# Firstastor/polars-quant

Hardware: AMD Instinct MI355X
Metric: indicator+backtest rows/sec, 5000 sym x 2520 day f64 OHLCV (higher is better)
Workload: dtype f64

## Files before the change

polars_quant_amd/csrc/pattern.hip:

```cpp
#include "pq_dev.h"

struct Cdl {
    double o, h, l, c;
    double body, us, ls, mx, mn;
    bool bull, bear, lng, sht, doji, lus, lds, sus, sds, vsus, vsds, vlds;
    __device__ void set(double o_, double h_, double l_, double c_) {
        o = o_; h = h_; l = l_; c = c_;
        bull = c > o;
        bear = c < o;
        body = fabs(o - c);
        mn = fmin(o, c);
        mx = fmax(o, c);
        us = h - mx;
        ls = mn - l;
        lng = body > 0.05 * (o + c) * 0.5;
        sht = body < 0.1 * (o + c) * 0.5;
        doji = body <= 0.005 * (o + c) * 0.5;
        lus = us > 2.0 * body;
        lds = ls > 2.0 * body;
        sus = us < 0.5 * body;
        sds = ls < 0.5 * body;
        vsus = us < 0.1 * body;
        vsds = ls < 0.1 * body;
        vlds = ls > 3.0 * body;
    }
    __device__ bool maru() const { return lng && vsus && vsds; }
};
__device__ __forceinline__ bool nearq(double a, double b, const Cdl &k) { return fabs(a - b) < 0.01 * (k.h + k.l) * 0.5; }
__device__ __forceinline__ bool equalq(double a, double b, const Cdl &k) { return fabs(a - b) < 0.001 * (k.h + k.l) * 0.5; }
__device__ __forceinline__ int pm(bool up, bool dn) { return up ? 100 : (dn ? -100 : 0); }

__device__ __forceinline__ int cdl_eval(int id, const Cdl &a, const Cdl &b, const Cdl &c, const Cdl &d, const Cdl &e, double pen,
                                        int *lookback) {
    switch (id) {
    case 0: *lookback = 2;
        return (c.bull & c.lng & b.bear & b.o > c.c & a.bear & a.o > b.o & a.o < b.c & a.c > c.o & a.c < c.c) ? -100 : 0;
    case 1: *lookback = 2;
        return (c.bear & c.lng & b.bear & b.lng & a.bear & a.lng & b.o < c.o & b.o > c.c & a.o < b.o & a.o > b.c &
                b.c < c.c & a.c < b.c) ? -100 : 0;
    case 2: *lookback = 2;
        return pm(c.bear & c.lng & b.bull & b.c < c.o & b.o > c.c & a.bull & a.c > c.o,
                  c.bull & c.lng & b.bear & b.o < c.c & b.c > c.o & a.bear & a.c < c.o);
    case 3: *lookback = 3;
        return pm(d.bear & c.bear & b.bear & c.c < d.c & b.c < c.c & c.o > d.c & c.o < d.o & b.o > c.c & b.o < c.o &
                      a.bull & a.o < b.c & a.c > d.o,
                  d.bull & c.bull & b.bull & c.c > d.c & b.c > c.c & c.o < d.c & c.o > d.o & b.o < c.c & b.o > c.o &
                      a.bear & a.o > b.c & a.c < d.o);
    case 4: *lookback = 2;
        return pm(c.bear & b.bull & b.o <= c.c & b.c >= c.o & a.bull & a.c > b.c,
                  c.bull & b.bear & b.o >= c.c & b.c <= c.o & a.bear & a.c < b.c);
    case 5: *lookback = 2;
        return (c.bear & c.lng & c.lds & b.bear & b.l > c.l & b.c > c.c & a.bear & a.sht & a.h < b.h & a.l > b.l) ? 100 : 0;
    case 6: *lookback = 2;
        return (c.bull & c.lng & b.bull & b.lng & a.bull & a.lng & b.o > c.o & b.o <= c.c & a.o > b.o & a.o <= b.c &
                b.c > c.c & a.c > b.c) ? 100 : 0;
    case 7: *lookback = 2;
        return pm(c.bear & c.lng & b.doji & b.h < c.l & a.bull & a.l > b.h,
                  c.bull & c.lng & b.doji & b.l > c.h & a.bear & a.h < b.l);
    case 8: *lookback = 2;
        return (c.bull & c.lng & b.bull & a.bull & b.o > c.o & b.o <= c.c & a.o > b.o & a.o <= b.c & b.c > c.c &
                a.c > b.c & a.body < b.body) ? -100 : 0;
    case 9: *lookback = 0;
        return pm(a.bull & a.lng & a.vsds, a.bear & a.lng & a.vsus);
    case 10: *lookback = 4;
        return pm(e.bear & e.lng & d.bear & d.o < e.c & c.c < d.c & a.bull & a.c > d.o & a.c < e.c,
                  e.bull & e.lng & d.bull & d.o > e.c & c.c > d.c & a.bear & a.c < d.o & a.c > e.c);
    case 11: *lookback = 0;
        return pm(a.bull & a.lng & a.vsus, a.bear & a.lng & a.vsds);
    case 12: *lookback = 3;
        return (d.bear & d.lng & d.vsus & d.vsds & c.bear & c.lng & c.vsus & c.vsds & c.c < d.c & b.bear &
                b.h > c.c & a.bear & a.lng & a.o > b.h & a.c < c.l) ? 100 : 0;
    case 13: *lookback = 1;
        return pm(b.bear & b.lng & a.bull & a.lng & nearq(a.c, b.c, a), b.bull & b.lng & a.bear & a.lng & nearq(a.c, b.c, a));
    case 14: *lookback = 1;
        return (b.bull & b.lng & a.bear & a.o > b.c & a.c < (b.c - (b.body * pen)) & a.c > b.o) ? -100 : 0;
    case 15: *lookback = 0;
        return a.doji ? 100 : 0;
    case 16: { *lookback = 1;
        double mid = (a.o + a.c) / 2.0;
        return pm(b.bear & b.lng & a.doji & mid < b.c, b.bull & b.lng & a.doji & mid > b.c); }
    case 17: *lookback = 0;
        return (a.doji & a.lds & a.vsus) ? 100 : 0;
    case 18: *lookback = 1;
        return pm(b.bear & a.bull & a.o <= b.c & a.c >= b.o & (a.o < b.c | a.c > b.o),
                  b.bull & a.bear & a.o >= b.c & a.c <= b.o & (a.o > b.c | a.c < b.o));
    case 19: *lookback = 2;
        return (c.bull & c.lng & b.doji & b.mn > c.c & a.bear & a.c < (c.c - (c.body * pen))) ? -100 : 0;
    case 20: *lookback = 2;
        return (c.bull & c.lng & b.sht & b.mn > c.c & a.bear & a.c < (c.c - (c.body * pen))) ? -100 : 0;
    case 21: { *lookback = 2;
        bool common = b.bull & a.bull & nearq(a.body, b.body, a) & nearq(a.o, b.o, a);
        return pm(c.bull & b.o > c.c & common, c.bear & b.c < c.c & common); }
    case 22: *lookback = 0;
        return (a.doji & a.lus & a.vsds) ? -100 : 0;
    case 23: *lookback = 1;
        return (a.sht & a.ls > (2.0 * a.body) & a.vsus & b.bear) ? 100 : 0;
    case 24: *lookback = 1;
        return (a.sht & a.ls > (2.0 * a.body) & a.vsus & b.bull) ? -100 : 0;
    case 25: *lookback = 1;
        return pm(b.bear & b.lng & a.bull & a.sht & a.o > b.c & a.c < b.o, b.bull & b.lng & a.bear & a.sht & a.o < b.c & a.c > b.o);
    case 26: *lookback = 1;
        return pm(b.bear & b.lng & a.doji & a.mx < b.o & a.mn > b.c, b.bull & b.lng & a.doji & a.mx < b.c & a.mn > b.o);
    case 27: { *lookback = 0;
        bool m = a.sht & a.lus & a.lds;
        return pm(m & a.bull, m & a.bear); }
    case 28: { *lookback = 2;
        bool inside = b.h < c.h & b.l > c.l;
        return pm(inside & a.c > c.h & a.bull, inside & a.c < c.l & a.bear); }
    case 29: { *lookback = 3;
        bool inside = c.h < d.h & c.l > d.l & b.h < c.h & b.l > c.l;
        return pm(inside & a.c > d.h & a.bull, inside & a.c < d.l & a.bear); }
    case 30: *lookback = 1;
        return (b.bear & b.lng & a.bear & a.sht & a.o < b.o & a.c > b.c) ? 100 : 0;
    case 31: *lookback = 2;
        return (c.bear & c.lng & b.bear & b.lng & a.bear & a.lng & equalq(b.o, c.c, a) & equalq(a.o, b.c, a) &
                b.c < c.c & a.c < b.c) ? -100 : 0;
    case 32: *lookback = 1;
        return (b.bear & b.lng & a.bull & a.o < b.c & nearq(a.c, b.c, a)) ? -100 : 0;
    case 33: *lookback = 1;
        return (a.sht & a.us > (2.0 * a.body) & a.vsds & b.bear) ? 100 : 0;
    case 34: *lookback = 1;
        return pm(b.bear & b.maru() & a.bull & a.maru() & a.o > b.o, b.bull & b.maru() & a.bear & a.maru() & a.o < b.o);
    case 35: { *lookback = 1;
        bool bk = b.bear & b.maru() & a.bull & a.maru() & a.o > b.o;
        bool sk = b.bull & b.maru() & a.bear & a.maru() & a.o < b.o;
        bool longer = a.body >= b.body;
        bool bl = bk & longer, sl = sk & longer;
        return pm(bl | (bk & !sl), sl | (sk & !bl)); }
    case 36: *lookback = 4;
        return (e.bear & e.lng & d.bear & d.c < e.c & c.bear & c.c < d.c & b.bear & b.lus & a.bull & a.o > b.o) ? 100 : 0;
    case 37: *lookback = 0;
        return (a.doji & a.lus & a.lds) ? 100 : 0;
    case 38: { *lookback = 0;
        bool m = a.lng & a.sus & a.sds;
        return pm(m & a.bull, m & a.bear); }
    case 39: { *lookback = 0;
        bool m = a.maru();
        return pm(m & a.bull, m & a.bear); }
    case 40: *lookback = 1;
        return (b.bear & b.lng & a.bear & equalq(a.c, b.c, a)) ? 100 : 0;
    case 41: *lookback = 4;
        return (e.bull & e.lng & d.sht & d.o > e.c & c.sht & b.sht & d.l > e.o & c.l > e.o & b.l > e.o & a.bull &
                a.c > e.c) ? 100 : 0;
    case 42: *lookback = 2;
        return (c.bear & c.lng & b.doji & b.mx < c.c & a.bull & a.c > (c.c + (c.body * pen))) ? 100 : 0;
    case 43: *lookback = 2;
        return (c.bear & c.lng & b.sht & b.mx < c.c & a.bull & a.c > (c.c + (c.body * pen))) ? 100 : 0;
    case 44: *lookback = 1;
        return (b.bear & b.lng & a.bull & a.o < b.c & nearq(a.c, b.l, a)) ? -100 : 0;
    case 45: *lookback = 1;
        return (b.bear & b.lng & a.bull & a.o < b.c & a.c > (b.c + (b.body * pen)) & a.c < b.o) ? 100 : 0;
    case 46: *lookback = 0;
        return (a.doji & a.lus & a.lds & nearq(a.us, a.ls, a)) ? 100 : 0;
    case 47: { *lookback = 4;
        bool mid = d.sht & c.sht & b.sht & d.h < e.h & c.h < e.h & b.h < e.h & d.l > e.l & c.l > e.l & b.l > e.l;
        return pm(e.bull & e.lng & mid & a.bull & a.lng & a.c > e.c, e.bear & e.lng & mid & a.bear & a.lng & a.c < e.c); }
    case 48: *lookback = 1;
        return pm(b.bear & b.lng & a.bull & a.lng & equalq(a.o, b.o, a), b.bull & b.lng & a.bear & a.lng & equalq(a.o, b.o, a));
    case 49: *lookback = 1;
        return (a.sht & a.us > (2.0 * a.body) & a.vsds & b.bull) ? -100 : 0;
    case 50: { *lookback = 0;
        bool m = a.sht & a.sus & a.sds;
        return pm(m & a.bull, m & a.bear); }
    case 51: { *lookback = 0;
        bool m = a.sht & a.us > a.body & a.ls > a.body;
        return pm(m & a.bull, m & a.bear); }
    case 52: *lookback = 2;
        return (c.bull & c.lng & b.bull & b.lng & b.c > c.c & a.bull & a.sht & a.c > b.c & a.o > b.o & a.o <= b.c) ? -100 : 0;
    case 53: *lookback = 2;
        return (c.bear & c.lng & b.bull & b.lng & b.o > c.c & a.bear & a.lng & equalq(a.c, c.c, a)) ? 100 : 0;
    case 54: *lookback = 0;
        return (a.doji & a.vlds & a.vsus) ? 100 : 0;
    case 55: *lookback = 2;
        return pm(c.bull & b.bull & b.o > c.c & a.bear & a.o > b.o & a.o < b.c & a.c > c.o & a.c < c.c,
                  c.bear & b.bear & b.o < c.c & a.bull & a.o < b.o & a.o > b.c & a.c < c.o & a.c > c.c);
    case 56: { *lookback = 1;
        double midpoint = b.c + (b.body * 0.5);
        return (b.bear & b.lng & a.bull & a.o < b.c & a.c > b.c & a.c < midpoint) ? -100 : 0; }
    case 57: { *lookback = 2;
        bool dj = c.doji & b.doji & a.doji;
        double m1 = (c.o + c.c) / 2.0, m2 = (b.o + b.c) / 2.0, m3 = (a.o + a.c) / 2.0;
        return pm(dj & m2 < m1 & m3 > m2, dj & m2 > m1 & m3 < m2); }
    case 58: *lookback = 2;
        return (c.bear & c.lng & b.bear & b.l < c.l & b.c > b.l & b.o < c.o & b.o > c.c & a.bull & a.sht & a.c < b.c) ? 100 : 0;
    case 59: *lookback = 2;
        return (c.bull & c.lng & b.bear & b.o > c.c & b.c > c.c & a.bear & a.o > b.o & a.c > c.c & a.c < b.c) ? -100 : 0;
    case 60: *lookback = 2;
        return pm(c.bull & b.bull & b.o > c.c & a.bear & a.o < b.c & a.o > b.o & a.c > c.o & a.c < c.c,
                  c.bear & b.bear & b.o < c.c & a.bull & a.o > b.c & a.o < b.o & a.c < c.o & a.c > c.c);
    }
    *lookback = 0;
    return 0;
}

struct CdlArgs {
    const double *o, *h, *l, *c;
    int32_t *out[PQ_N_PATTERNS];
    double pen[PQ_N_PATTERNS];
};

__device__ __forceinline__ Cdl load_candle(const CdlArgs &a, int64_t base, int64_t q) {
    Cdl k;
    if (q >= 0) k.set(a.o[base + q], a.h[base + q], a.l[base + q], a.c[base + q]);
    else k.set(0.0, 0.0, 0.0, 0.0);
    return k;
}

#ifndef PQ_CDL_R
#define PQ_CDL_R 1
#endif
constexpr int CDL_R = PQ_CDL_R;
template <bool ALL, bool VEC>
__global__ __launch_bounds__(ROW_BLOCK) void cdl_all_kernel(CdlArgs a, Dims d) {
    const int64_t s = blockIdx.y;
    const int64_t t0 = ((int64_t)blockIdx.x * ROW_BLOCK + threadIdx.x) * CDL_R;
    const int64_t slen = dims_len(d, s);
    if (t0 >= slen) return;
    const int64_t base = dims_base(d, s);
#ifndef PQ_CDL_PRIO
#define PQ_CDL_PRIO 0
#endif
    __builtin_amdgcn_s_setprio(PQ_CDL_PRIO);
    Cdl w[CDL_R + 4];
#pragma unroll
    for (int k = 0; k < CDL_R + 4; k++) {
        const int64_t q = t0 + CDL_R - 1 - k;
        w[k] = load_candle(a, base, q < slen ? q : slen - 1);
    }
#pragma unroll
    for (int id = 0; id < PQ_N_PATTERNS; id++) {
        if (!ALL && a.out[id] == nullptr) continue;
        int v[CDL_R];
#pragma unroll
        for (int r = 0; r < CDL_R; r++) {
            int lb;
            const int x = cdl_eval(id, w[CDL_R - 1 - r], w[CDL_R - r], w[CDL_R + 1 - r], w[CDL_R + 2 - r], w[CDL_R + 3 - r], a.pen[id], &lb);
            v[r] = (t0 + r >= lb) ? x : 0;
        }
#if PQ_EXP_NOSTORE_ON
        if (v[0] == 123456789) a.out[id][base + t0] = v[0];
#else
        int32_t *dst = &a.out[id][base + t0];
        if (VEC && (CDL_R == 1 || t0 + CDL_R <= slen)) {
            typedef int pq_irv __attribute__((ext_vector_type(CDL_R)));
            pq_irv vv;
#pragma unroll
            for (int r = 0; r < CDL_R; r++) vv[r] = v[r];
            __builtin_nontemporal_store(vv, reinterpret_cast<pq_irv *>(dst));
        } else {
#pragma unroll
            for (int r = 0; r < CDL_R; r++)
                if (t0 + r < slen) __builtin_nontemporal_store(v[r], dst + r);
        }
#endif
    }
}

__global__ __launch_bounds__(ROW_BLOCK) void cdl_one_kernel(CdlArgs a, int id, Dims d) {
    const int64_t s = blockIdx.y;
    const int64_t t = (int64_t)blockIdx.x * ROW_BLOCK + threadIdx.x;
    if (t >= dims_len(d, s)) return;
    const int64_t base = dims_base(d, s);
    Cdl w[5];
#pragma unroll
    for (int k = 0; k < 5; k++) w[k] = load_candle(a, base, t - k);
    int lb;
    int v = cdl_eval(id, w[0], w[1], w[2], w[3], w[4], a.pen[0], &lb);
    a.out[0][base + t] = (t >= lb) ? v : 0;
}

static const char *const k_pattern_names[PQ_N_PATTERNS] = {
    "cdl2crows", "cdl3blackcrows", "cdl3inside", "cdl3linestrike", "cdl3outside", "cdl3starsinsouth",
    "cdl3whitesoldiers", "cdlabandonedbaby", "cdladvanceblock", "cdlbelthold", "cdlbreakaway",
    "cdlclosingmarubozu", "cdlconcealbabyswall", "cdlcounterattack", "cdldarkcloudcover", "cdldoji",
    "cdldojistar", "cdldragonflydoji", "cdlengulfing", "cdleveningdojistar", "cdleveningstar",
    "cdlgapsidesidewhite", "cdlgravestonedoji", "cdlhammer", "cdlhangingman", "cdlharami", "cdlharamicross",
    "cdlhighwave", "cdlhikkake", "cdlhikkakemod", "cdlhomingpigeon", "cdlidentical3crows", "cdlinneck",
    "cdlinvertedhammer", "cdlkicking", "cdlkickingbylength", "cdlladderbottom", "cdllongleggeddoji",
    "cdllongline", "cdlmarubozu", "cdlmatchinglow", "cdlmathold", "cdlmorningdojistar", "cdlmorningstar",
    "cdlonneck", "cdlpiercing", "cdlrickshawman", "cdlrisefall3methods", "cdlseparatinglines",
    "cdlshootingstar", "cdlshortline", "cdlspinningtop", "cdlstalledpattern", "cdlsticksandwich", "cdltakuri",
    "cdltasukigap", "cdlthrusting", "cdltristar", "cdlunique3river", "cdlupsidegap2crows",
    "cdlxsidegap3methods"};

#include <string.h>
extern "C" {

const char *pq_pattern_name(int32_t id) { return (id >= 0 && id < PQ_N_PATTERNS) ? k_pattern_names[id] : nullptr; }
int32_t pq_pattern_id(const char *name) {
    if (!name) return -1;
    for (int i = 0; i < PQ_N_PATTERNS; i++)
        if (strcmp(name, k_pattern_names[i]) == 0) return i;
    return -1;
}

struct CdlBlob {
    CdlArgs args;
    int id;
    pq_batch b;
};
static void cdl_launch_blob(const void *blob, hipStream_t stream);
static pq_status cdl_launch(pq_ctx *ctx, const pq_batch *b, const CdlArgs &args, int id) {
    if (b->n_series == 0 || b->len == 0) return PQ_OK;
    CdlBlob cb{args, id, *b};
    if (ctx->rec) {
        static_assert(sizeof(CdlBlob) <= sizeof(RowThunk::blob), "CdlBlob too large");
        RowThunk t;
        t.launch = &cdl_launch_blob;
        t.row_id = 0;
        t.blob_bytes = (int)sizeof cb;
        t.dims = dims_of(b);
        memcpy(t.blob, &cb, sizeof cb);
        t.n_reads = 4;
        t.reads[0] = args.o; t.reads[1] = args.h; t.reads[2] = args.l; t.reads[3] = args.c;
        t.n_writes = 0;
        for (int i = 0; i < PQ_N_PATTERNS; i++) if (args.out[i]) t.writes[t.n_writes++] = args.out[i];
        return rec_add_row(ctx, t);
    }
    cdl_launch_blob(&cb, ctx->stream);
    PQ_HIP_TRY(hipGetLastError());
    return PQ_OK;
}
static void cdl_launch_blob(const void *blob, hipStream_t stream) {
    const CdlBlob &cb = *reinterpret_cast<const CdlBlob *>(blob);
    const pq_batch *b = &cb.b;
    const CdlArgs &args = cb.args;
    const int id = cb.id;
    for (int64_t s0 = 0; s0 < b->n_series; s0 += 65535) {
        int64_t ns = b->n_series - s0 < 65535 ? b->n_series - s0 : 65535;
        CdlArgs a2 = args;
        int64_t off = b->offsets ? 0 : s0 * b->stride;
        a2.o += off; a2.h += off; a2.l += off; a2.c += off;
        for (int i = 0; i < PQ_N_PATTERNS; i++) if (a2.out[i]) a2.out[i] += off;
        dim3 grid((unsigned)((b->len + ROW_BLOCK - 1) / ROW_BLOCK), (unsigned)ns);
        Dims d{ns, b->len, b->stride, b->offsets ? b->offsets + s0 : nullptr};
        if (id < 0) {
            int vec = (b->stride % CDL_R) == 0 && !b->offsets;
            for (int i = 0; i < PQ_N_PATTERNS; i++)
                if (a2.out[i] && reinterpret_cast<uintptr_t>(a2.out[i]) % (4 * CDL_R)) vec = 0;
            const int64_t per_block = (int64_t)ROW_BLOCK * CDL_R;
            dim3 grid2((unsigned)((b->len + per_block - 1) / per_block), (unsigned)ns);
            bool all = true;
            for (int i = 0; i < PQ_N_PATTERNS; i++) all &= a2.out[i] != nullptr;
            if (all && vec) hipLaunchKernelGGL((cdl_all_kernel<true, true>), grid2, dim3(ROW_BLOCK), 0, stream, a2, d);
            else if (all) hipLaunchKernelGGL((cdl_all_kernel<true, false>), grid2, dim3(ROW_BLOCK), 0, stream, a2, d);
            else if (vec) hipLaunchKernelGGL((cdl_all_kernel<false, true>), grid2, dim3(ROW_BLOCK), 0, stream, a2, d);
            else hipLaunchKernelGGL((cdl_all_kernel<false, false>), grid2, dim3(ROW_BLOCK), 0, stream, a2, d);
        } else hipLaunchKernelGGL(cdl_one_kernel, grid, dim3(ROW_BLOCK), 0, stream, a2, id, d);
    }
}

pq_status pq_cdl(pq_ctx *ctx, const pq_batch *b, int32_t id, const double *o, const double *h, const double *l,
                 const double *c, double penetration, int32_t *out) {
    PQ_TRY(pq_check(ctx, b));
    PQ_REQUIRE(o && h && l && c && out, "pq_cdl: null pointer");
    PQ_REQUIRE(id >= 0 && id < PQ_N_PATTERNS, "pq_cdl: pattern id out of range");
    CdlArgs a;
    memset(&a, 0, sizeof a);
    a.o = o; a.h = h; a.l = l; a.c = c;
    a.out[0] = out; a.pen[0] = penetration;
    return cdl_launch(ctx, b, a, id);
}

pq_status pq_cdl_all(pq_ctx *ctx, const pq_batch *b, const double *o, const double *h, const double *l,
                     const double *c, const double *penetrations, int32_t *const *outs) {
    PQ_TRY(pq_check(ctx, b));
    PQ_REQUIRE(o && h && l && c && penetrations && outs, "pq_cdl_all: null pointer");
    CdlArgs a;
    memset(&a, 0, sizeof a);
    a.o = o; a.h = h; a.l = l; a.c = c;
    for (int i = 0; i < PQ_N_PATTERNS; i++) { a.out[i] = outs[i]; a.pen[i] = penetrations[i]; }
    return cdl_launch(ctx, b, a, -1);
}

}
```

Before: 3.741 billion.

## Recompute candle flags lazily and restructure pattern emission with scalar address staging

Candle boolean flags are no longer stored per candle but computed on demand, which cuts live per-candle state and register pressure. Patterns are emitted in a compile-time order grouped by lookback, with scheduling barriers between them. Output column pointers are prefetched from the kernarg segment in batches of four, and a wave-uniform base address is built with readfirstlane so each lane adds only a small byte offset. The host permutes the output and penetration arrays to match the new order. In exchange, shared flag comparisons may be recomputed across patterns, and the code relies on fragile inline-asm and address-space tricks.

```diff
diff --git a/polars_quant_amd/csrc/pattern.hip b/polars_quant_amd/csrc/pattern.hip
--- a/polars_quant_amd/csrc/pattern.hip
+++ b/polars_quant_amd/csrc/pattern.hip
@@ -1,30 +1,30 @@
 #include "pq_dev.h"
+#include <utility>
 
 struct Cdl {
     double o, h, l, c;
     double body, us, ls, mx, mn;
-    bool bull, bear, lng, sht, doji, lus, lds, sus, sds, vsus, vsds, vlds;
     __device__ void set(double o_, double h_, double l_, double c_) {
         o = o_; h = h_; l = l_; c = c_;
-        bull = c > o;
-        bear = c < o;
         body = fabs(o - c);
         mn = fmin(o, c);
         mx = fmax(o, c);
         us = h - mx;
         ls = mn - l;
-        lng = body > 0.05 * (o + c) * 0.5;
-        sht = body < 0.1 * (o + c) * 0.5;
-        doji = body <= 0.005 * (o + c) * 0.5;
-        lus = us > 2.0 * body;
-        lds = ls > 2.0 * body;
-        sus = us < 0.5 * body;
-        sds = ls < 0.5 * body;
-        vsus = us < 0.1 * body;
-        vsds = ls < 0.1 * body;
-        vlds = ls > 3.0 * body;
-    }
-    __device__ bool maru() const { return lng && vsus && vsds; }
+    }
+    __device__ __forceinline__ bool bull() const { return c > o; }
+    __device__ __forceinline__ bool bear() const { return c < o; }
+    __device__ __forceinline__ bool lng() const { return body > 0.05 * (o + c) * 0.5; }
+    __device__ __forceinline__ bool sht() const { return body < 0.1 * (o + c) * 0.5; }
+    __device__ __forceinline__ bool doji() const { return body <= 0.005 * (o + c) * 0.5; }
+    __device__ __forceinline__ bool lus() const { return us > 2.0 * body; }
+    __device__ __forceinline__ bool lds() const { return ls > 2.0 * body; }
+    __device__ __forceinline__ bool sus() const { return us < 0.5 * body; }
+    __device__ __forceinline__ bool sds() const { return ls < 0.5 * body; }
+    __device__ __forceinline__ bool vsus() const { return us < 0.1 * body; }
+    __device__ __forceinline__ bool vsds() const { return ls < 0.1 * body; }
+    __device__ __forceinline__ bool vlds() const { return ls > 3.0 * body; }
+    __device__ __forceinline__ bool maru() const { return lng() & vsus() & vsds(); }
 };
 __device__ __forceinline__ bool nearq(double a, double b, const Cdl &k) { return fabs(a - b) < 0.01 * (k.h + k.l) * 0.5; }
 __device__ __forceinline__ bool equalq(double a, double b, const Cdl &k) { return fabs(a - b) < 0.001 * (k.h + k.l) * 0.5; }
@@ -34,160 +34,160 @@
                                         int *lookback) {
     switch (id) {
     case 0: *lookback = 2;
-        return (c.bull & c.lng & b.bear & b.o > c.c & a.bear & a.o > b.o & a.o < b.c & a.c > c.o & a.c < c.c) ? -100 : 0;
+        return (c.bull() & c.lng() & b.bear() & b.o > c.c & a.bear() & a.o > b.o & a.o < b.c & a.c > c.o & a.c < c.c) ? -100 : 0;
     case 1: *lookback = 2;
-        return (c.bear & c.lng & b.bear & b.lng & a.bear & a.lng & b.o < c.o & b.o > c.c & a.o < b.o & a.o > b.c &
+        return (c.bear() & c.lng() & b.bear() & b.lng() & a.bear() & a.lng() & b.o < c.o & b.o > c.c & a.o < b.o & a.o > b.c &
                 b.c < c.c & a.c < b.c) ? -100 : 0;
     case 2: *lookback = 2;
-        return pm(c.bear & c.lng & b.bull & b.c < c.o & b.o > c.c & a.bull & a.c > c.o,
-                  c.bull & c.lng & b.bear & b.o < c.c & b.c > c.o & a.bear & a.c < c.o);
+        return pm(c.bear() & c.lng() & b.bull() & b.c < c.o & b.o > c.c & a.bull() & a.c > c.o,
+                  c.bull() & c.lng() & b.bear() & b.o < c.c & b.c > c.o & a.bear() & a.c < c.o);
     case 3: *lookback = 3;
-        return pm(d.bear & c.bear & b.bear & c.c < d.c & b.c < c.c & c.o > d.c & c.o < d.o & b.o > c.c & b.o < c.o &
-                      a.bull & a.o < b.c & a.c > d.o,
-                  d.bull & c.bull & b.bull & c.c > d.c & b.c > c.c & c.o < d.c & c.o > d.o & b.o < c.c & b.o > c.o &
-                      a.bear & a.o > b.c & a.c < d.o);
+        return pm(d.bear() & c.bear() & b.bear() & c.c < d.c & b.c < c.c & c.o > d.c & c.o < d.o & b.o > c.c & b.o < c.o &
+                      a.bull() & a.o < b.c & a.c > d.o,
+                  d.bull() & c.bull() & b.bull() & c.c > d.c & b.c > c.c & c.o < d.c & c.o > d.o & b.o < c.c & b.o > c.o &
+                      a.bear() & a.o > b.c & a.c < d.o);
     case 4: *lookback = 2;
-        return pm(c.bear & b.bull & b.o <= c.c & b.c >= c.o & a.bull & a.c > b.c,
-                  c.bull & b.bear & b.o >= c.c & b.c <= c.o & a.bear & a.c < b.c);
+        return pm(c.bear() & b.bull() & b.o <= c.c & b.c >= c.o & a.bull() & a.c > b.c,
+                  c.bull() & b.bear() & b.o >= c.c & b.c <= c.o & a.bear() & a.c < b.c);
     case 5: *lookback = 2;
-        return (c.bear & c.lng & c.lds & b.bear & b.l > c.l & b.c > c.c & a.bear & a.sht & a.h < b.h & a.l > b.l) ? 100 : 0;
+        return (c.bear() & c.lng() & c.lds() & b.bear() & b.l > c.l & b.c > c.c & a.bear() & a.sht() & a.h < b.h & a.l > b.l) ? 100 : 0;
     case 6: *lookback = 2;
-        return (c.bull & c.lng & b.bull & b.lng & a.bull & a.lng & b.o > c.o & b.o <= c.c & a.o > b.o & a.o <= b.c &
+        return (c.bull() & c.lng() & b.bull() & b.lng() & a.bull() & a.lng() & b.o > c.o & b.o <= c.c & a.o > b.o & a.o <= b.c &
                 b.c > c.c & a.c > b.c) ? 100 : 0;
     case 7: *lookback = 2;
-        return pm(c.bear & c.lng & b.doji & b.h < c.l & a.bull & a.l > b.h,
-                  c.bull & c.lng & b.doji & b.l > c.h & a.bear & a.h < b.l);
+        return pm(c.bear() & c.lng() & b.doji() & b.h < c.l & a.bull() & a.l > b.h,
+                  c.bull() & c.lng() & b.doji() & b.l > c.h & a.bear() & a.h < b.l);
     case 8: *lookback = 2;
-        return (c.bull & c.lng & b.bull & a.bull & b.o > c.o & b.o <= c.c & a.o > b.o & a.o <= b.c & b.c > c.c &
+        return (c.bull() & c.lng() & b.bull() & a.bull() & b.o > c.o & b.o <= c.c & a.o > b.o & a.o <= b.c & b.c > c.c &
                 a.c > b.c & a.body < b.body) ? -100 : 0;
     case 9: *lookback = 0;
-        return pm(a.bull & a.lng & a.vsds, a.bear & a.lng & a.vsus);
+        return pm(a.bull() & a.lng() & a.vsds(), a.bear() & a.lng() & a.vsus());
     case 10: *lookback = 4;
-        return pm(e.bear & e.lng & d.bear & d.o < e.c & c.c < d.c & a.bull & a.c > d.o & a.c < e.c,
-                  e.bull & e.lng & d.bull & d.o > e.c & c.c > d.c & a.bear & a.c < d.o & a.c > e.c);
+        return pm(e.bear() & e.lng() & d.bear() & d.o < e.c & c.c < d.c & a.bull() & a.c > d.o & a.c < e.c,
+                  e.bull() & e.lng() & d.bull() & d.o > e.c & c.c > d.c & a.bear() & a.c < d.o & a.c > e.c);
     case 11: *lookback = 0;
-        return pm(a.bull & a.lng & a.vsus, a.bear & a.lng & a.vsds);
+        return pm(a.bull() & a.lng() & a.vsus(), a.bear() & a.lng() & a.vsds());
     case 12: *lookback = 3;
-        return (d.bear & d.lng & d.vsus & d.vsds & c.bear & c.lng & c.vsus & c.vsds & c.c < d.c & b.bear &
-                b.h > c.c & a.bear & a.lng & a.o > b.h & a.c < c.l) ? 100 : 0;
+        return (d.bear() & d.lng() & d.vsus() & d.vsds() & c.bear() & c.lng() & c.vsus() & c.vsds() & c.c < d.c & b.bear() &
+                b.h > c.c & a.bear() & a.lng() & a.o > b.h & a.c < c.l) ? 100 : 0;
     case 13: *lookback = 1;
-        return pm(b.bear & b.lng & a.bull & a.lng & nearq(a.c, b.c, a), b.bull & b.lng & a.bear & a.lng & nearq(a.c, b.c, a));
+        return pm(b.bear() & b.lng() & a.bull() & a.lng() & nearq(a.c, b.c, a), b.bull() & b.lng() & a.bear() & a.lng() & nearq(a.c, b.c, a));
     case 14: *lookback = 1;
-        return (b.bull & b.lng & a.bear & a.o > b.c & a.c < (b.c - (b.body * pen)) & a.c > b.o) ? -100 : 0;
+        return (b.bull() & b.lng() & a.bear() & a.o > b.c & a.c < (b.c - (b.body * pen)) & a.c > b.o) ? -100 : 0;
     case 15: *lookback = 0;
-        return a.doji ? 100 : 0;
+        return a.doji() ? 100 : 0;
     case 16: { *lookback = 1;
         double mid = (a.o + a.c) / 2.0;
-        return pm(b.bear & b.lng & a.doji & mid < b.c, b.bull & b.lng & a.doji & mid > b.c); }
+        return pm(b.bear() & b.lng() & a.doji() & mid < b.c, b.bull() & b.lng() & a.doji() & mid > b.c); }
     case 17: *lookback = 0;
-        return (a.doji & a.lds & a.vsus) ? 100 : 0;
+        return (a.doji() & a.lds() & a.vsus()) ? 100 : 0;
     case 18: *lookback = 1;
-        return pm(b.bear & a.bull & a.o <= b.c & a.c >= b.o & (a.o < b.c | a.c > b.o),
-                  b.bull & a.bear & a.o >= b.c & a.c <= b.o & (a.o > b.c | a.c < b.o));
+        return pm(b.bear() & a.bull() & a.o <= b.c & a.c >= b.o & (a.o < b.c | a.c > b.o),
+                  b.bull() & a.bear() & a.o >= b.c & a.c <= b.o & (a.o > b.c | a.c < b.o));
     case 19: *lookback = 2;
-        return (c.bull & c.lng & b.doji & b.mn > c.c & a.bear & a.c < (c.c - (c.body * pen))) ? -100 : 0;
+        return (c.bull() & c.lng() & b.doji() & b.mn > c.c & a.bear() & a.c < (c.c - (c.body * pen))) ? -100 : 0;
     case 20: *lookback = 2;
-        return (c.bull & c.lng & b.sht & b.mn > c.c & a.bear & a.c < (c.c - (c.body * pen))) ? -100 : 0;
+        return (c.bull() & c.lng() & b.sht() & b.mn > c.c & a.bear() & a.c < (c.c - (c.body * pen))) ? -100 : 0;
     case 21: { *lookback = 2;
-        bool common = b.bull & a.bull & nearq(a.body, b.body, a) & nearq(a.o, b.o, a);
-        return pm(c.bull & b.o > c.c & common, c.bear & b.c < c.c & common); }
+        bool common = b.bull() & a.bull() & nearq(a.body, b.body, a) & nearq(a.o, b.o, a);
+        return pm(c.bull() & b.o > c.c & common, c.bear() & b.c < c.c & common); }
     case 22: *lookback = 0;
-        return (a.doji & a.lus & a.vsds) ? -100 : 0;
+        return (a.doji() & a.lus() & a.vsds()) ? -100 : 0;
     case 23: *lookback = 1;
-        return (a.sht & a.ls > (2.0 * a.body) & a.vsus & b.bear) ? 100 : 0;
+        return (a.sht() & a.ls > (2.0 * a.body) & a.vsus() & b.bear()) ? 100 : 0;
     case 24: *lookback = 1;
-        return (a.sht & a.ls > (2.0 * a.body) & a.vsus & b.bull) ? -100 : 0;
+        return (a.sht() & a.ls > (2.0 * a.body) & a.vsus() & b.bull()) ? -100 : 0;
     case 25: *lookback = 1;
-        return pm(b.bear & b.lng & a.bull & a.sht & a.o > b.c & a.c < b.o, b.bull & b.lng & a.bear & a.sht & a.o < b.c & a.c > b.o);
+        return pm(b.bear() & b.lng() & a.bull() & a.sht() & a.o > b.c & a.c < b.o, b.bull() & b.lng() & a.bear() & a.sht() & a.o < b.c & a.c > b.o);
     case 26: *lookback = 1;
-        return pm(b.bear & b.lng & a.doji & a.mx < b.o & a.mn > b.c, b.bull & b.lng & a.doji & a.mx < b.c & a.mn > b.o);
+        return pm(b.bear() & b.lng() & a.doji() & a.mx < b.o & a.mn > b.c, b.bull() & b.lng() & a.doji() & a.mx < b.c & a.mn > b.o);
     case 27: { *lookback = 0;
-        bool m = a.sht & a.lus & a.lds;
-        return pm(m & a.bull, m & a.bear); }
+        bool m = a.sht() & a.lus() & a.lds();
+        return pm(m & a.bull(), m & a.bear()); }
     case 28: { *lookback = 2;
         bool inside = b.h < c.h & b.l > c.l;
-        return pm(inside & a.c > c.h & a.bull, inside & a.c < c.l & a.bear); }
+        return pm(inside & a.c > c.h & a.bull(), inside & a.c < c.l & a.bear()); }
     case 29: { *lookback = 3;
         bool inside = c.h < d.h & c.l > d.l & b.h < c.h & b.l > c.l;
-        return pm(inside & a.c > d.h & a.bull, inside & a.c < d.l & a.bear); }
+        return pm(inside & a.c > d.h & a.bull(), inside & a.c < d.l & a.bear()); }
     case 30: *lookback = 1;
-        return (b.bear & b.lng & a.bear & a.sht & a.o < b.o & a.c > b.c) ? 100 : 0;
+        return (b.bear() & b.lng() & a.bear() & a.sht() & a.o < b.o & a.c > b.c) ? 100 : 0;
     case 31: *lookback = 2;
-        return (c.bear & c.lng & b.bear & b.lng & a.bear & a.lng & equalq(b.o, c.c, a) & equalq(a.o, b.c, a) &
+        return (c.bear() & c.lng() & b.bear() & b.lng() & a.bear() & a.lng() & equalq(b.o, c.c, a) & equalq(a.o, b.c, a) &
                 b.c < c.c & a.c < b.c) ? -100 : 0;
     case 32: *lookback = 1;
-        return (b.bear & b.lng & a.bull & a.o < b.c & nearq(a.c, b.c, a)) ? -100 : 0;
+        return (b.bear() & b.lng() & a.bull() & a.o < b.c & nearq(a.c, b.c, a)) ? -100 : 0;
     case 33: *lookback = 1;
-        return (a.sht & a.us > (2.0 * a.body) & a.vsds & b.bear) ? 100 : 0;
+        return (a.sht() & a.us > (2.0 * a.body) & a.vsds() & b.bear()) ? 100 : 0;
     case 34: *lookback = 1;
-        return pm(b.bear & b.maru() & a.bull & a.maru() & a.o > b.o, b.bull & b.maru() & a.bear & a.maru() & a.o < b.o);
+        return pm(b.bear() & b.maru() & a.bull() & a.maru() & a.o > b.o, b.bull() & b.maru() & a.bear() & a.maru() & a.o < b.o);
     case 35: { *lookback = 1;
-        bool bk = b.bear & b.maru() & a.bull & a.maru() & a.o > b.o;
-        bool sk = b.bull & b.maru() & a.bear & a.maru() & a.o < b.o;
+        bool bk = b.bear() & b.maru() & a.bull() & a.maru() & a.o > b.o;
+        bool sk = b.bull() & b.maru() & a.bear() & a.maru() & a.o < b.o;
         bool longer = a.body >= b.body;
         bool bl = bk & longer, sl = sk & longer;
         return pm(bl | (bk & !sl), sl | (sk & !bl)); }
     case 36: *lookback = 4;
-        return (e.bear & e.lng & d.bear & d.c < e.c & c.bear & c.c < d.c & b.bear & b.lus & a.bull & a.o > b.o) ? 100 : 0;
+        return (e.bear() & e.lng() & d.bear() & d.c < e.c & c.bear() & c.c < d.c & b.bear() & b.lus() & a.bull() & a.o > b.o) ? 100 : 0;
     case 37: *lookback = 0;
-        return (a.doji & a.lus & a.lds) ? 100 : 0;
+        return (a.doji() & a.lus() & a.lds()) ? 100 : 0;
     case 38: { *lookback = 0;
-        bool m = a.lng & a.sus & a.sds;
-        return pm(m & a.bull, m & a.bear); }
+        bool m = a.lng() & a.sus() & a.sds();
+        return pm(m & a.bull(), m & a.bear()); }
     case 39: { *lookback = 0;
         bool m = a.maru();
-        return pm(m & a.bull, m & a.bear); }
+        return pm(m & a.bull(), m & a.bear()); }
     case 40: *lookback = 1;
-        return (b.bear & b.lng & a.bear & equalq(a.c, b.c, a)) ? 100 : 0;
+        return (b.bear() & b.lng() & a.bear() & equalq(a.c, b.c, a)) ? 100 : 0;
     case 41: *lookback = 4;
-        return (e.bull & e.lng & d.sht & d.o > e.c & c.sht & b.sht & d.l > e.o & c.l > e.o & b.l > e.o & a.bull &
+        return (e.bull() & e.lng() & d.sht() & d.o > e.c & c.sht() & b.sht() & d.l > e.o & c.l > e.o & b.l > e.o & a.bull() &
                 a.c > e.c) ? 100 : 0;
     case 42: *lookback = 2;
-        return (c.bear & c.lng & b.doji & b.mx < c.c & a.bull & a.c > (c.c + (c.body * pen))) ? 100 : 0;
+        return (c.bear() & c.lng() & b.doji() & b.mx < c.c & a.bull() & a.c > (c.c + (c.body * pen))) ? 100 : 0;
     case 43: *lookback = 2;
-        return (c.bear & c.lng & b.sht & b.mx < c.c & a.bull & a.c > (c.c + (c.body * pen))) ? 100 : 0;
+        return (c.bear() & c.lng() & b.sht() & b.mx < c.c & a.bull() & a.c > (c.c + (c.body * pen))) ? 100 : 0;
     case 44: *lookback = 1;
-        return (b.bear & b.lng & a.bull & a.o < b.c & nearq(a.c, b.l, a)) ? -100 : 0;
+        return (b.bear() & b.lng() & a.bull() & a.o < b.c & nearq(a.c, b.l, a)) ? -100 : 0;
     case 45: *lookback = 1;
-        return (b.bear & b.lng & a.bull & a.o < b.c & a.c > (b.c + (b.body * pen)) & a.c < b.o) ? 100 : 0;
+        return (b.bear() & b.lng() & a.bull() & a.o < b.c & a.c > (b.c + (b.body * pen)) & a.c < b.o) ? 100 : 0;
     case 46: *lookback = 0;
-        return (a.doji & a.lus & a.lds & nearq(a.us, a.ls, a)) ? 100 : 0;
+        return (a.doji() & a.lus() & a.lds() & nearq(a.us, a.ls, a)) ? 100 : 0;
     case 47: { *lookback = 4;
-        bool mid = d.sht & c.sht & b.sht & d.h < e.h & c.h < e.h & b.h < e.h & d.l > e.l & c.l > e.l & b.l > e.l;
-        return pm(e.bull & e.lng & mid & a.bull & a.lng & a.c > e.c, e.bear & e.lng & mid & a.bear & a.lng & a.c < e.c); }
+        bool mid = d.sht() & c.sht() & b.sht() & d.h < e.h & c.h < e.h & b.h < e.h & d.l > e.l & c.l > e.l & b.l > e.l;
+        return pm(e.bull() & e.lng() & mid & a.bull() & a.lng() & a.c > e.c, e.bear() & e.lng() & mid & a.bear() & a.lng() & a.c < e.c); }
     case 48: *lookback = 1;
-        return pm(b.bear & b.lng & a.bull & a.lng & equalq(a.o, b.o, a), b.bull & b.lng & a.bear & a.lng & equalq(a.o, b.o, a));
+        return pm(b.bear() & b.lng() & a.bull() & a.lng() & equalq(a.o, b.o, a), b.bull() & b.lng() & a.bear() & a.lng() & equalq(a.o, b.o, a));
     case 49: *lookback = 1;
-        return (a.sht & a.us > (2.0 * a.body) & a.vsds & b.bull) ? -100 : 0;
+        return (a.sht() & a.us > (2.0 * a.body) & a.vsds() & b.bull()) ? -100 : 0;
     case 50: { *lookback = 0;
-        bool m = a.sht & a.sus & a.sds;
-        return pm(m & a.bull, m & a.bear); }
+        bool m = a.sht() & a.sus() & a.sds();
+        return pm(m & a.bull(), m & a.bear()); }
     case 51: { *lookback = 0;
-        bool m = a.sht & a.us > a.body & a.ls > a.body;
-        return pm(m & a.bull, m & a.bear); }
+        bool m = a.sht() & a.us > a.body & a.ls > a.body;
+        return pm(m & a.bull(), m & a.bear()); }
     case 52: *lookback = 2;
-        return (c.bull & c.lng & b.bull & b.lng & b.c > c.c & a.bull & a.sht & a.c > b.c & a.o > b.o & a.o <= b.c) ? -100 : 0;
+        return (c.bull() & c.lng() & b.bull() & b.lng() & b.c > c.c & a.bull() & a.sht() & a.c > b.c & a.o > b.o & a.o <= b.c) ? -100 : 0;
     case 53: *lookback = 2;
-        return (c.bear & c.lng & b.bull & b.lng & b.o > c.c & a.bear & a.lng & equalq(a.c, c.c, a)) ? 100 : 0;
+        return (c.bear() & c.lng() & b.bull() & b.lng() & b.o > c.c & a.bear() & a.lng() & equalq(a.c, c.c, a)) ? 100 : 0;
     case 54: *lookback = 0;
-        return (a.doji & a.vlds & a.vsus) ? 100 : 0;
+        return (a.doji() & a.vlds() & a.vsus()) ? 100 : 0;
     case 55: *lookback = 2;
-        return pm(c.bull & b.bull & b.o > c.c & a.bear & a.o > b.o & a.o < b.c & a.c > c.o & a.c < c.c,
-                  c.bear & b.bear & b.o < c.c & a.bull & a.o < b.o & a.o > b.c & a.c < c.o & a.c > c.c);
+        return pm(c.bull() & b.bull() & b.o > c.c & a.bear() & a.o > b.o & a.o < b.c & a.c > c.o & a.c < c.c,
+                  c.bear() & b.bear() & b.o < c.c & a.bull() & a.o < b.o & a.o > b.c & a.c < c.o & a.c > c.c);
     case 56: { *lookback = 1;
         double midpoint = b.c + (b.body * 0.5);
-        return (b.bear & b.lng & a.bull & a.o < b.c & a.c > b.c & a.c < midpoint) ? -100 : 0; }
+        return (b.bear() & b.lng() & a.bull() & a.o < b.c & a.c > b.c & a.c < midpoint) ? -100 : 0; }
     case 57: { *lookback = 2;
-        bool dj = c.doji & b.doji & a.doji;
+        bool dj = c.doji() & b.doji() & a.doji();
         double m1 = (c.o + c.c) / 2.0, m2 = (b.o + b.c) / 2.0, m3 = (a.o + a.c) / 2.0;
         return pm(dj & m2 < m1 & m3 > m2, dj & m2 > m1 & m3 < m2); }
     case 58: *lookback = 2;
-        return (c.bear & c.lng & b.bear & b.l < c.l & b.c > b.l & b.o < c.o & b.o > c.c & a.bull & a.sht & a.c < b.c) ? 100 : 0;
+        return (c.bear() & c.lng() & b.bear() & b.l < c.l & b.c > b.l & b.o < c.o & b.o > c.c & a.bull() & a.sht() & a.c < b.c) ? 100 : 0;
     case 59: *lookback = 2;
-        return (c.bull & c.lng & b.bear & b.o > c.c & b.c > c.c & a.bear & a.o > b.o & a.c > c.c & a.c < b.c) ? -100 : 0;
+        return (c.bull() & c.lng() & b.bear() & b.o > c.c & b.c > c.c & a.bear() & a.o > b.o & a.c > c.c & a.c < b.c) ? -100 : 0;
     case 60: *lookback = 2;
-        return pm(c.bull & b.bull & b.o > c.c & a.bear & a.o < b.c & a.o > b.o & a.c > c.o & a.c < c.c,
-                  c.bear & b.bear & b.o < c.c & a.bull & a.o > b.c & a.o < b.o & a.c < c.o & a.c > c.c);
+        return pm(c.bull() & b.bull() & b.o > c.c & a.bear() & a.o < b.c & a.o > b.o & a.c > c.o & a.c < c.c,
+                  c.bear() & b.bear() & b.o < c.c & a.bull() & a.o > b.c & a.o < b.o & a.c < c.o & a.c > c.c);
     }
     *lookback = 0;
     return 0;
@@ -210,6 +210,95 @@
 #define PQ_CDL_R 1
 #endif
 constexpr int CDL_R = PQ_CDL_R;
+
+constexpr int k_cdl_order[PQ_N_PATTERNS] = {
+    10, 36, 41, 47,
+    3, 12, 29,
+    0, 1, 2, 4, 5, 6, 7, 8, 19, 20, 21, 28, 31, 42, 43, 52, 53, 55, 57, 58, 59, 60,
+    13, 14, 16, 18, 23, 24, 25, 26, 30, 32, 33, 34, 35, 40, 44, 45, 48, 49, 56,
+    9, 11, 15, 17, 22, 27, 37, 38, 39, 46, 50, 51, 54};
+constexpr bool cdl_order_is_permutation() {
+    bool seen[PQ_N_PATTERNS] = {};
+    for (int id : k_cdl_order) {
+        if (id < 0 || id >= PQ_N_PATTERNS || seen[id]) return false;
+        seen[id] = true;
+    }
+    return true;
+}
+static_assert(cdl_order_is_permutation(), "k_cdl_order names every recogniser exactly once");
+
+typedef __attribute__((address_space(1))) int pq_gint;
+typedef __attribute__((address_space(1))) unsigned char pq_gbyte1;
+struct CdlRows {
+    int64_t rows0;
+    unsigned lane_b;
+    int64_t t0, slen;
+    bool ge[CDL_R][5];
+};
+#ifndef PQ_CDL_PB
+#define PQ_CDL_PB 4
+#endif
+constexpr int CDL_PB = PQ_CDL_PB;
+typedef __attribute__((address_space(4))) const CdlArgs pq_cdl_kargs;
+struct CdlCols {
+    pq_cdl_kargs *ka;
+    int32_t *cur[CDL_PB], *nxt[CDL_PB];
+    template <int K0>
+    __device__ __forceinline__ void fetch() {
+        asm volatile("" : "+s"(ka));
+#pragma unroll
+        for (int j = 0; j < CDL_PB; j++) nxt[j] = K0 + j < PQ_N_PATTERNS ? ka->out[K0 + j] : nullptr;
+    }
+    template <int K>
+    __device__ __forceinline__ void advance() {
+        if constexpr (K % CDL_PB == 0) {
+#pragma unroll
+            for (int j = 0; j < CDL_PB; j++) cur[j] = nxt[j];
+            if constexpr (K + CDL_PB < PQ_N_PATTERNS) fetch<K + CDL_PB>();
+        }
+    }
+};
+template <int K, bool ALL, bool VEC>
+__device__ __forceinline__ void cdl_emit(const CdlArgs &a, CdlCols &cols, const Cdl (&w)[CDL_R + 4], const CdlRows &g) {
+    constexpr int ID = k_cdl_order[K];
+    cols.template advance<K>();
+    int32_t *const col = cols.cur[K % CDL_PB];
+    if (!ALL && col == nullptr) return;
+    int v[CDL_R];
+#pragma unroll
+    for (int r = 0; r < CDL_R; r++) {
+        int lb;
+        const int x = cdl_eval(ID, w[CDL_R - 1 - r], w[CDL_R - r], w[CDL_R + 1 - r], w[CDL_R + 2 - r], w[CDL_R + 3 - r], a.pen[K], &lb);
+        v[r] = g.ge[r][lb] ? x : 0;
+    }
+    const unsigned long long p = reinterpret_cast<unsigned long long>(col + g.rows0);
+    unsigned lo = __builtin_amdgcn_readfirstlane((unsigned)p), hi = __builtin_amdgcn_readfirstlane((unsigned)(p >> 32));
+    asm("" : "+s"(lo), "+s"(hi));
+    unsigned off = g.lane_b;
+    asm volatile("" : "+v"(off));
+    pq_gint *dst = (pq_gint *)((pq_gbyte1 *)(((unsigned long long)hi << 32) | lo) + off);
+#if PQ_EXP_NOSTORE_ON
+    if (v[0] == 123456789) *dst = v[0];
+#else
+    if (VEC && (CDL_R == 1 || g.t0 + CDL_R <= g.slen)) {
+        typedef int pq_irv __attribute__((ext_vector_type(CDL_R)));
+        typedef __attribute__((address_space(1))) pq_irv pq_girv;
+        pq_irv vv;
+#pragma unroll
+        for (int r = 0; r < CDL_R; r++) vv[r] = v[r];
+        __builtin_nontemporal_store(vv, (pq_girv *)dst);
+    } else {
+#pragma unroll
+        for (int r = 0; r < CDL_R; r++)
+            if (g.t0 + r < g.slen) __builtin_nontemporal_store(v[r], dst + r);
+    }
+#endif
+}
+template <bool ALL, bool VEC, int... KS>
+__device__ __forceinline__ void cdl_emit_all(const CdlArgs &a, CdlCols &cols, const Cdl (&w)[CDL_R + 4], const CdlRows &g, std::integer_sequence<int, KS...>) {
+    ((cdl_emit<KS, ALL, VEC>(a, cols, w, g), __builtin_amdgcn_sched_barrier(0)), ...);
+}
+
 template <bool ALL, bool VEC>
 __global__ __launch_bounds__(ROW_BLOCK) void cdl_all_kernel(CdlArgs a, Dims d) {
     const int64_t s = blockIdx.y;
@@ -221,39 +310,26 @@
 #define PQ_CDL_PRIO 0
 #endif
     __builtin_amdgcn_s_setprio(PQ_CDL_PRIO);
+    CdlCols cols;
+    cols.ka = (pq_cdl_kargs *)__builtin_amdgcn_kernarg_segment_ptr();
+    cols.template fetch<0>();
     Cdl w[CDL_R + 4];
 #pragma unroll
     for (int k = 0; k < CDL_R + 4; k++) {
         const int64_t q = t0 + CDL_R - 1 - k;
         w[k] = load_candle(a, base, q < slen ? q : slen - 1);
     }
-#pragma unroll
-    for (int id = 0; id < PQ_N_PATTERNS; id++) {
-        if (!ALL && a.out[id] == nullptr) continue;
-        int v[CDL_R];
-#pragma unroll
-        for (int r = 0; r < CDL_R; r++) {
-            int lb;
-            const int x = cdl_eval(id, w[CDL_R - 1 - r], w[CDL_R - r], w[CDL_R + 1 - r], w[CDL_R + 2 - r], w[CDL_R + 3 - r], a.pen[id], &lb);
-            v[r] = (t0 + r >= lb) ? x : 0;
-        }
-#if PQ_EXP_NOSTORE_ON
-        if (v[0] == 123456789) a.out[id][base + t0] = v[0];
-#else
-        int32_t *dst = &a.out[id][base + t0];
-        if (VEC && (CDL_R == 1 || t0 + CDL_R <= slen)) {
-            typedef int pq_irv __attribute__((ext_vector_type(CDL_R)));
-            pq_irv vv;
-#pragma unroll
-            for (int r = 0; r < CDL_R; r++) vv[r] = v[r];
-            __builtin_nontemporal_store(vv, reinterpret_cast<pq_irv *>(dst));
-        } else {
-#pragma unroll
-            for (int r = 0; r < CDL_R; r++)
-                if (t0 + r < slen) __builtin_nontemporal_store(v[r], dst + r);
-        }
-#endif
-    }
+    CdlRows g;
+    const unsigned wave_row0 = __builtin_amdgcn_readfirstlane(threadIdx.x & ~63u);
+    g.rows0 = base + ((int64_t)blockIdx.x * ROW_BLOCK + wave_row0) * CDL_R;
+    g.lane_b = (threadIdx.x & 63u) * (unsigned)(4 * CDL_R);
+    g.t0 = t0;
+    g.slen = slen;
+#pragma unroll
+    for (int r = 0; r < CDL_R; r++)
+#pragma unroll
+        for (int lb = 0; lb < 5; lb++) g.ge[r][lb] = t0 + r >= lb;
+    cdl_emit_all<ALL, VEC>(a, cols, w, g, std::make_integer_sequence<int, PQ_N_PATTERNS>{});
 }
 
 __global__ __launch_bounds__(ROW_BLOCK) void cdl_one_kernel(CdlArgs a, int id, Dims d) {
@@ -369,7 +445,7 @@
     CdlArgs a;
     memset(&a, 0, sizeof a);
     a.o = o; a.h = h; a.l = l; a.c = c;
-    for (int i = 0; i < PQ_N_PATTERNS; i++) { a.out[i] = outs[i]; a.pen[i] = penetrations[i]; }
+    for (int k = 0; k < PQ_N_PATTERNS; k++) { a.out[k] = outs[k_cdl_order[k]]; a.pen[k] = penetrations[k_cdl_order[k]]; }
     return cdl_launch(ctx, b, a, -1);
 }
 
```

Result: faster. 3.917 billion, median of 6 (+4.7%).
